# WeeFav/Visual-Odometry-GPU

Measured on AMD Instinct MI355X. Metric: ORB detect+describe frames/sec (1241x376, 8 lvls), higher is better.
Workload: dtype u8; 1 GPU; KITTI-shaped 1241x376 u8, 8 levels s=1.2, 1000 features, FAST-9 t=20, NMS 3x3, Harris top-N, blur5 all levels, BRIEF-256; batch=1024 frames/step/GPU resident in HBM (stream A); distinct_resident_batches=2, fast_early_exit=True, pyramid_blur_fused=True, pyramid_top_rows_first=True, pipelined_batches=True

## Files before the change

visual-odometry-gpu_amd/csrc/orbx_kernels.hip:

```cpp
#include <hip/hip_runtime.h>

#include <cstdlib>

#include "orbx_internal.h"
#include "orbx_math.h"
#include "orbx_wave.h"

__constant__ __attribute__((aligned(16))) int8_t c_pattern[1024] = {
#include "pattern_31.inc"
};


typedef uint16_t __attribute__((aligned(1))) u16_unaligned;

__device__ __forceinline__ void decode_tile(const OrbxTileMap& tm, int nlevels, int& l, int& tx, int& ty) {
  const int t = blockIdx.x;
  l = 0;
#pragma unroll 1
  for (int i = 1; i < nlevels; i++)
    if (t >= tm.begin[i]) l = i;
  const int local = t - tm.begin[l];
  ty = local / tm.tiles_x[l];
  tx = local - ty * tm.tiles_x[l];
}
// ... 705 lines not shown
  const size_t co = (size_t)f * plan.cand_total + L.cand_off;
  const int n8 = (n + 7) & ~7;
  for (int i = tid; i < n8; i += 256) {
    u64 key = 0ull;
    if (i < n) {
      uint32_t u = orbx_f2u(resp[co + i]);
      if (u == 0x80000000u) u = 0u;
      u ^= (u >> 31) ? 0xffffffffu : 0x80000000u;
      key = ((u64)u << 32) | (uint32_t)~(uint32_t)i;
    }
    s_key[i] = key;
  }
  __syncthreads();
  const int ci = tid & (RANK_SLICE - 1), part = tid >> 6;
  const int i = first + ci;
  const u64 ki = s_key[i < n8 ? i : 0];
  const int per = n8 / 4;
  int rank = 0;
  for (int j = part * per; j < (part + 1) * per; j += 2) {
    const ulonglong2 v = *reinterpret_cast<const ulonglong2*>(&s_key[j]);
    rank += v.x > ki;
    rank += v.y > ki;
  }
  s_part[part][ci] = rank;
  __syncthreads();
  if (part == 0 && i < n) {
    rank = s_part[0][ci] + s_part[1][ci] + s_part[2][ci] + s_part[3][ci];
    if (rank < keep) {
      const uint32_t p = cand[co + i];
      const size_t so = (size_t)f * plan.out_cap + L.out_off;
      orbx_keypoint kp;
      kp.x = (int)(p & 0xffffu);
      kp.y = (int)(p >> 16);
      sel_lkp[so + rank] = kp;
      sel_resp[so + rank] = resp[co + i];
    }
  }
}

__global__ __launch_bounds__(256) void k_select_flat(const float* __restrict__ resp, int n, int keep,
                                                     int32_t* __restrict__ idx) {
  const int m = n < keep ? n : keep;
  for (int i = blockIdx.x * 256 + threadIdx.x; i < n; i += gridDim.x * 256) {
    const float ri = resp[i];
    int rank = 0;
    for (int j = 0; j < n; j++) {
      const float rj = resp[j];
      rank += (rj > ri) || (rj == ri && j < i);
    }
    if (rank < m) idx[rank] = i;
  }
}

#define DESC_R 20
#define DESC_ROWS (2 * DESC_R + 1)
#define DESC_PITCH 48
#define DESC_HP 40
#define DESC_BROWS (DESC_ROWS - 4)

struct DescLds {
  union {
    uint32_t patch[DESC_ROWS * DESC_PITCH / 4];
    uint16_t box[DESC_BROWS * DESC_HP];
  };
  uint16_t hs[DESC_ROWS * DESC_HP];
};

__device__ __forceinline__ u64 hsum5x4(uint32_t d0, uint32_t d1) {
  const u64 acc = (u64)__builtin_amdgcn_perm(d1, d1, 0x0c010c00u) |
                  ((u64)__builtin_amdgcn_perm(d1, d1, 0x0c030c02u) << 32);
  return __builtin_amdgcn_qsad_pk_u16_u8((u64)d0 | ((u64)d1 << 32), 0u, acc);
}

struct DescJob {
  const uint8_t* img;
  int w, h, pitch;
  int x, y;
  bool valid;
};

__device__ __forceinline__ void describe_wave(const DescJob& jb, DescLds& lds, int patch_size,
                                              bool use_given_angle, float given_angle, bool do_brief,
                                              float& angle_out, u64 desc_out[4]) {
  const int lane = lane_id();
  const uint8_t* s_patch = reinterpret_cast<const uint8_t*>(lds.patch);
  const int px0 = jb.x - DESC_R, py0 = jb.y - DESC_R;
  const int ax0 = px0 & ~3;
  const int off = px0 - ax0;
  if (jb.valid) {
    int row = lane / (DESC_PITCH / 4), c = lane - row * (DESC_PITCH / 4);
#pragma unroll
    for (int k = 0; k < (DESC_ROWS * (DESC_PITCH / 4) + 63) / 64; k++) {
      const int i = lane + 64 * k;
      if (i < DESC_ROWS * (DESC_PITCH / 4)) {
        const int gy = py0 + row, gx = ax0 + 4 * c;
        uint32_t v = 0;
        if ((unsigned)gy < (unsigned)jb.h && (unsigned)gx < (unsigned)jb.pitch)
          v = *reinterpret_cast<const uint32_t*>(jb.img + (uint32_t)(gy * jb.pitch + gx));
        lds.patch[i] = v;
      }
      row += 5;
      c += 4;
      if (c >= DESC_PITCH / 4) {
        c -= DESC_PITCH / 4;
        row += 1;
      }
    }
  }
  __syncthreads();
  float angle = 0.0f;
  if (jb.valid) {
    if (use_given_angle) {
      angle = given_angle;
    } else {
      const int pr = patch_size / 2, P = 2 * pr + 1;
      if (!(jb.x - pr < 0 || jb.x + pr >= jb.w || jb.y - pr < 0 || jb.y + pr >= jb.h)) {
        const int grp_shift = P <= 32 ? 5 : 6;
        const int col = lane & ((1 << grp_shift) - 1), grp = lane >> grp_shift, ngrp = 64 >> grp_shift;
        int colsum = 0, m01 = 0;
        if (col < P) {
          const uint8_t* pc = s_patch + (DESC_R - pr) * DESC_PITCH + (col - pr + DESC_R + off);
          for (int rr = grp; rr < P; rr += ngrp) {
            const int I = pc[rr * DESC_PITCH];
            colsum += I;
            m01 += (rr - pr) * I;
          }
        }
        int m10 = (col - pr) * colsum;
        m10 = wave_sum(m10);
        m01 = wave_sum(m01);
        angle = orbx_atan2f((float)m01, (float)m10);
      }
    }
  }
  angle_out = angle;
  if (!do_brief) return;

  if (jb.valid) {
    int r = lane / 10, g = lane - r * 10;
#pragma unroll
    for (int k = 0; k < (DESC_ROWS * 10 + 63) / 64; k++) {
      if (lane + 64 * k < DESC_ROWS * 10) {
        const uint32_t d0 = lds.patch[r * (DESC_PITCH / 4) + g], d1 = lds.patch[r * (DESC_PITCH / 4) + g + 1];
        *reinterpret_cast<u64*>(&lds.hs[r * DESC_HP + 4 * g]) = hsum5x4(d0, d1);
      }
      r += 6;
      g += 4;
      if (g >= 10) {
        g -= 10;
        r += 1;
      }
    }
  }
  __syncthreads();
  if (jb.valid) {
    int r = lane / 10, g = lane - r * 10;
#pragma unroll
    for (int k = 0; k < (DESC_BROWS * 10 + 63) / 64; k++) {
      if (lane + 64 * k < DESC_BROWS * 10) {
        const uint2* hp = reinterpret_cast<const uint2*>(&lds.hs[r * DESC_HP + 4 * g]);
        uint2 acc = hp[0];
#pragma unroll
        for (int q = 1; q < 5; q++) {
          const uint2 v = hp[q * (DESC_HP / 4)];
          acc.x = pk_add(acc.x, v.x);
          acc.y = pk_add(acc.y, v.y);
        }
        *reinterpret_cast<uint2*>(&lds.box[r * DESC_HP + 4 * g]) = acc;
      }
      r += 6;
      g += 4;
      if (g >= 10) {
        g -= 10;
        r += 1;
      }
    }
  }
  __syncthreads();

  const float c = orbx_cosf(angle), s = orbx_sinf(angle);
#pragma unroll 1
  for (int k = 0; k < 4; k++) {
    bool bit = false;
    if (jb.valid) {
      const int i = k * 64 + lane;
      const int32_t pk = reinterpret_cast<const int32_t*>(c_pattern)[i];
      const float x1 = (float)(int8_t)(pk & 0xff), y1 = (float)(int8_t)((pk >> 8) & 0xff);
      const float x2 = (float)(int8_t)((pk >> 16) & 0xff), y2 = (float)(int8_t)((pk >> 24) & 0xff);
      int dx1 = orbx_lroundf(__fsub_rn(__fmul_rn(c, x1), __fmul_rn(s, y1)));
      int dy1 = orbx_lroundf(__fadd_rn(__fmul_rn(s, x1), __fmul_rn(c, y1)));
      int dx2 = orbx_lroundf(__fsub_rn(__fmul_rn(c, x2), __fmul_rn(s, y2)));
      int dy2 = orbx_lroundf(__fadd_rn(__fmul_rn(s, x2), __fmul_rn(c, y2)));
      const int cx1 = jb.x + dx1, cy1 = jb.y + dy1, cx2 = jb.x + dx2, cy2 = jb.y + dy2;
      const bool skip = cx1 < 2 || cy1 < 2 || cx1 > jb.w - 1 || cy1 > jb.h - 1 || cx2 < 2 || cy2 < 2 ||
                        cx2 > jb.w - 1 || cy2 > jb.h - 1;
      if (!skip) {
        dx1 = min(max(dx1, -18), 18);
        dy1 = min(max(dy1, -18), 18);
        dx2 = min(max(dx2, -18), 18);
        dy2 = min(max(dy2, -18), 18);
        const int s1 = lds.box[(dy1 + 18) * DESC_HP + dx1 + 18 + off];
        const int s2 = lds.box[(dy2 + 18) * DESC_HP + dx2 + 18 + off];
        bit = s1 < s2;
      }
    }
    desc_out[k] = __ballot(bit);
  }
}



#define DESC_NLD ((DESC_ROWS * (DESC_PITCH / 4) + 63) / 64)

__device__ __forceinline__ void desc_fetch_patch(const DescJob& jb, int lane, uint32_t (&regs)[DESC_NLD],
                                                 int& off_out) {
  const int px0 = jb.x - DESC_R, py0 = jb.y - DESC_R;
  const int ax0 = px0 & ~3;
  off_out = px0 - ax0;
  int row = lane / (DESC_PITCH / 4), c = lane - row * (DESC_PITCH / 4);
#pragma unroll
  for (int k = 0; k < DESC_NLD; k++) {
    const int gy = py0 + row, gx = ax0 + 4 * c;
    uint32_t v = 0;
    if (lane + 64 * k < DESC_ROWS * (DESC_PITCH / 4) && (unsigned)gy < (unsigned)jb.h &&
        (unsigned)gx < (unsigned)jb.pitch)
      v = *reinterpret_cast<const uint32_t*>(jb.img + (uint32_t)(gy * jb.pitch + gx));
    regs[k] = v;
    row += 5;
    c += 4;
    if (c >= DESC_PITCH / 4) {
      c -= DESC_PITCH / 4;
      row += 1;
    }
  }
}

struct DescLds2 {
  uint32_t patch[DESC_ROWS * DESC_PITCH / 4];
  uint16_t hs[DESC_ROWS * DESC_HP];
};

template <class L>
__device__ __forceinline__ void desc_store_patch(L& lds, int lane, const uint32_t (&regs)[DESC_NLD]) {
#pragma unroll
  for (int k = 0; k < DESC_NLD; k++)
    if (lane + 64 * k < DESC_ROWS * (DESC_PITCH / 4)) lds.patch[lane + 64 * k] = regs[k];
}

__device__ __forceinline__ DescJob desc_job(const OrbxPlan& plan, const uint8_t* pyr, int f, orbx_keypoint kp,
                                            int level) {
  const OrbxLevel& L = plan.L[level];
  DescJob jb;
  jb.img = pyr + (size_t)f * plan.frame_bytes + L.img_off;
  jb.w = L.w;
  jb.h = L.h;
  jb.pitch = L.pitch;
  jb.x = kp.x;
  jb.y = kp.y;
  jb.valid = true;
  return jb;
}

template <class L>
__device__ __forceinline__ void desc_box_table_fused(L& lds, int lane) {
  static_assert(DESC_BROWS == 37, "6 chunks: 7 + 5 x 6 rows");
  const int chunk = lane / 10, g = lane - chunk * 10;
  if (chunk < 6) {
    const int r0 = chunk == 0 ? 0 : 6 * chunk + 1, nrows = chunk == 0 ? 7 : 6;
    const uint32_t* pp = &lds.patch[r0 * (DESC_PITCH / 4) + g];
    uint2* bp = reinterpret_cast<uint2*>(&lds.hs[r0 * DESC_HP + 4 * g]);
    auto hrow = [&](int i) {
      const u64 v = hsum5x4(pp[i * (DESC_PITCH / 4)], pp[i * (DESC_PITCH / 4) + 1]);
      return make_uint2((uint32_t)v, (uint32_t)(v >> 32));
    };
    uint2 q[5];
#pragma unroll
    for (int i = 0; i < 5; i++) q[i] = hrow(i);
    uint2 acc;
    acc.x = pk_add(pk_add(pk_add(q[0].x, q[1].x), pk_add(q[2].x, q[3].x)), q[4].x);
    acc.y = pk_add(pk_add(pk_add(q[0].y, q[1].y), pk_add(q[2].y, q[3].y)), q[4].y);
    bp[0] = acc;
#pragma unroll
    for (int i = 1; i < 7; i++) {
      if (i < nrows) {
        const uint2 nw = hrow(i + 4);
        const uint2 od = q[(i - 1) % 5];
        acc.x = pk_sub(pk_add(acc.x, nw.x), od.x);
        acc.y = pk_sub(pk_add(acc.y, nw.y), od.y);
        q[(i - 1) % 5] = nw;
        bp[i * (DESC_HP / 4)] = acc;
      }
    }
  }
  wave_lds_sync();
}

__device__ __forceinline__ float lround_f(float v) {
  const float t = __builtin_truncf(v);
  const float fr = __fsub_rn(v, t);
  return __fadd_rn(t, __builtin_truncf(__fadd_rn(fr, fr)));
}

typedef float f2_t __attribute__((ext_vector_type(2)));
__device__ __forceinline__ f2_t lround_f2(f2_t v) {
  const f2_t t = __builtin_elementwise_trunc(v);
  const f2_t fr = v - t;
  return t + __builtin_elementwise_trunc(fr + fr);
}

template <int DESC_KPW, int DESC_NW, int DESC_OCC>
__global__ __launch_bounds__(64 * DESC_NW, DESC_OCC) void k_describe2(OrbxPlan plan, const uint8_t* __restrict__ pyr, int patch_size,
                                                   const int32_t* __restrict__ sel_count,
                                                   const orbx_keypoint* __restrict__ sel_lkp,
                                                   const float* __restrict__ sel_resp,
                                                   int32_t* __restrict__ out_count,
                                                   orbx_keypoint* __restrict__ out_lkp,
                                                   float* __restrict__ out_resp,
                                                   int32_t* __restrict__ out_level,
                                                   orbx_keypoint* __restrict__ out_kp,
                                                   uint32_t* __restrict__ out_kp16,
                                                   float* __restrict__ out_angle,
                                                   orbx_descriptor* __restrict__ out_desc,
                                                   const uint32_t* __restrict__ feedback, uint32_t* __restrict__ feedback_host,
                                                   OrbxHostRecord host) {
  constexpr int DESC_KPB = DESC_NW * DESC_KPW;
  static_assert(2 * DESC_KPB <= 64 * DESC_NW, "trig: two threads per keypoint");
  __shared__ __attribute__((aligned(16))) DescLds2 s_lds[DESC_NW];
  __shared__ int s_m[DESC_KPB][2];
  __shared__ float s_cs[DESC_KPB][2];
  __shared__ uint2 s_mw[4 * (DESC_PITCH / 4)];
  __shared__ __attribute__((aligned(16))) uint32_t s_rec_kp[DESC_KPB], s_rec_angle[DESC_KPB], s_rec_desc[DESC_KPB][8];
  const int f = blockIdx.x, grp = blockIdx.y, tid = threadIdx.x, lane = tid & 63;
  const int wave = __builtin_amdgcn_readfirstlane(tid >> 6);
  static_assert(ORBX_MAX_LEVELS <= 64, "one lane per level");
  const int lvl_cnt = lane < plan.nlevels ? sel_count[f * plan.nlevels + lane] : 0;
  const int lvl_end = wave_scan_incl(lvl_cnt);
  const int count = __builtin_amdgcn_readlane(lvl_end, 63);
  if (grp == 0 && tid == 0) {
    out_count[f] = count;
    if (host.counts) host.counts[f] = count;
  }
  if (feedback_host && grp == 0 && f == 0 && tid < ORBX_FEEDBACK_WORDS) feedback_host[tid] = feedback[tid];
  const int slot0 = grp * DESC_KPB;
  if (slot0 >= count) return;
  DescLds2& lds = s_lds[wave];
  const int pr = patch_size / 2;
  if (tid < 4 * (DESC_PITCH / 4)) {
    const int off = tid / (DESC_PITCH / 4), c = tid - off * (DESC_PITCH / 4);
    uint32_t xw = 0, on = 0;
#pragma unroll
    for (int b = 0; b < 4; b++) {
      const int t = 4 * c + b - off - (DESC_R - pr);
      if (t >= 0 && t <= 2 * pr) {
        xw |= (uint32_t)t << (8 * b);
        on |= 1u << (8 * b);
      }
    }
    s_mw[tid] = make_uint2(xw, on);
  }
  int rowk[DESC_NLD], c3[3];
  uint32_t rin = 0;
  {
    int row = lane / (DESC_PITCH / 4), c = lane - row * (DESC_PITCH / 4);
#pragma unroll
    for (int k = 0; k < DESC_NLD; k++) {
      rowk[k] = row;
      if (k < 3) c3[k] = c;
      if (lane + 64 * k < DESC_ROWS * (DESC_PITCH / 4) && row >= DESC_R - pr && row <= DESC_R + pr) rin |= 1u << k;
      row += 5;
      c += 4;
      if (c >= DESC_PITCH / 4) {
        c -= DESC_PITCH / 4;
        row += 1;
      }
    }
  }
  __syncthreads();
  const size_t fo = (size_t)f * plan.out_cap;

  const int nk = min(DESC_KPW, max(0, count - (slot0 + wave * DESC_KPW)));
  DescJob jobs[DESC_KPW];
  float scale[DESC_KPW];
  uint32_t regs[DESC_KPW][DESC_NLD];
  int offs[DESC_KPW];
#pragma unroll
  for (int j = 0; j < DESC_KPW; j++) {
    const int slot = min(slot0 + wave * DESC_KPW + j, count - 1);
    const int level = __popcll(__ballot(lvl_end <= slot));
    const int lvl_begin = __builtin_amdgcn_readlane(lvl_end - lvl_cnt, level);
    const size_t src = fo + plan.L[level].out_off + (slot - lvl_begin);
    const orbx_keypoint kp = sel_lkp[src];
    jobs[j] = desc_job(plan, pyr, f, kp, level);
    scale[j] = plan.L[level].scale;
    if (j < nk && lane == 0) {
      out_lkp[fo + slot] = kp;
      out_resp[fo + slot] = sel_resp[src];
      out_level[fo + slot] = level;
    }
  }
#pragma unroll
  for (int j = 0; j < DESC_KPW; j++) {
    const DescJob& jb = jobs[j];
    const int py0 = jb.y - DESC_R, ax0 = (jb.x - DESC_R) & ~3;
    if (py0 >= 0 && py0 + DESC_ROWS <= jb.h && ax0 >= 0 && ax0 + DESC_PITCH <= jb.pitch) {
      offs[j] = jb.x - DESC_R - ax0;
      const uint32_t base = (uint32_t)(py0 * jb.pitch + ax0);
#pragma unroll
      for (int k = 0; k < DESC_NLD; k++) {
        regs[j][k] = 0;
        if (lane + 64 * k < DESC_ROWS * (DESC_PITCH / 4))
          regs[j][k] = *reinterpret_cast<const uint32_t*>(jb.img + (base + (__umul24((uint32_t)rowk[k], (uint32_t)jb.pitch) + 4u * (uint32_t)c3[k % 3])));
      }
    } else {
      desc_fetch_patch(jb, lane, regs[j], offs[j]);
    }
  }

#pragma unroll
  for (int j = 0; j < DESC_KPW; j++) {
    if (j < nk) {
      const DescJob& jb = jobs[j];
      const int q = wave * DESC_KPW + j, off = offs[j];
      int m10 = 0, m01 = 0;
      if (!(jb.x - pr < 0 || jb.x + pr >= jb.w || jb.y - pr < 0 || jb.y + pr >= jb.h)) {
        uint2 mw[3];
#pragma unroll
        for (int m = 0; m < 3; m++) mw[m] = s_mw[off * (DESC_PITCH / 4) + c3[m]];
        uint32_t X = 0, S = 0, M = 0;
#pragma unroll
        for (int k = 0; k < DESC_NLD; k++) {
          const uint32_t z = regs[j][k] & (uint32_t)(-(int32_t)((rin >> k) & 1u));
          X = __builtin_amdgcn_udot4(z, mw[k % 3].x, X, false);
          const uint32_t rs = __builtin_amdgcn_udot4(z, mw[k % 3].y, 0u, false);
          S += rs;
          M += __umul24((uint32_t)rowk[k], rs);
        }
        m10 = wave_sum((int)X - __mul24(pr, (int)S));
        m01 = wave_sum((int)M - __mul24(DESC_R, (int)S));
      }
      if (lane == 0) {
        s_m[q][0] = m10;
        s_m[q][1] = m01;
      }
    }
  }
  __syncthreads();
  if (tid < 2 * DESC_KPB && slot0 + (tid >> 1) < count) {
    const int q = tid >> 1, want_sin = tid & 1;
    const float angle = orbx_atan2f((float)s_m[q][1], (float)s_m[q][0]);
    s_cs[q][want_sin] = orbx_sincosf_impl(angle, want_sin ^ 1);
    if (!want_sin) {
      out_angle[fo + slot0 + q] = angle;
      s_rec_angle[q] = __float_as_uint(angle);
    }
  }
  __syncthreads();

  f2_t patx[4], paty[4];
#pragma unroll
  for (int k = 0; k < 4; k++) {
    const int32_t pk = reinterpret_cast<const int32_t*>(c_pattern)[k * 64 + lane];
    patx[k] = f2_t{(float)(int8_t)(pk & 0xff), (float)(int8_t)((pk >> 16) & 0xff)};
    paty[k] = f2_t{(float)(int8_t)((pk >> 8) & 0xff), (float)(int8_t)((pk >> 24) & 0xff)};
  }
#pragma unroll
  for (int j = 0; j < DESC_KPW; j++) {
    if (j < nk) {
      const DescJob& jb = jobs[j];
      const int q = wave * DESC_KPW + j, slot = slot0 + q, off = offs[j];
      desc_store_patch(lds, lane, regs[j]);
      wave_lds_sync();
      desc_box_table_fused(lds, lane);
      const float c = s_cs[q][0], s = s_cs[q][1];
      const bool interior = jb.x >= DESC_R && jb.y >= DESC_R && jb.x < jb.w - DESC_R && jb.y < jb.h - DESC_R;
      u64 d[4];
      if (interior) {
        const uint16_t* tbl = &lds.hs[18 * DESC_HP + 18 + off];
        const f2_t C2 = {c, c}, S2 = {s, s}, HP2 = {(float)DESC_HP, (float)DESC_HP};
#pragma unroll
        for (int k = 0; k < 4; k++) {
          const f2_t X = patx[k], Y = paty[k];
          const f2_t rx = lround_f2(C2 * X - S2 * Y), ry = lround_f2(S2 * X + C2 * Y);
          const f2_t idx = __builtin_elementwise_fma(ry, HP2, rx);
          d[k] = __ballot(tbl[(int)idx.x] < tbl[(int)idx.y]);
        }
      } else {
#pragma unroll
        for (int k = 0; k < 4; k++) {
          const float x1 = patx[k].x, y1 = paty[k].x, x2 = patx[k].y, y2 = paty[k].y;
          const int dx1 = orbx_lroundf(__fsub_rn(__fmul_rn(c, x1), __fmul_rn(s, y1)));
          const int dy1 = orbx_lroundf(__fadd_rn(__fmul_rn(s, x1), __fmul_rn(c, y1)));
          const int dx2 = orbx_lroundf(__fsub_rn(__fmul_rn(c, x2), __fmul_rn(s, y2)));
          const int dy2 = orbx_lroundf(__fadd_rn(__fmul_rn(s, x2), __fmul_rn(c, y2)));
          const int cx1 = jb.x + dx1, cy1 = jb.y + dy1, cx2 = jb.x + dx2, cy2 = jb.y + dy2;
          const bool ok = !(cx1 < 2 || cy1 < 2 || cx1 > jb.w - 1 || cy1 > jb.h - 1 || cx2 < 2 || cy2 < 2 ||
                            cx2 > jb.w - 1 || cy2 > jb.h - 1);
          const int s1 = lds.hs[(dy1 + 18) * DESC_HP + dx1 + 18 + off];
          const int s2 = lds.hs[(dy2 + 18) * DESC_HP + dx2 + 18 + off];
          d[k] = __ballot(ok && s1 < s2);
        }
      }
      wave_lds_sync();
      if (lane == 0) {
        orbx_keypoint g;
        g.x = (int)__fmul_rn((float)jb.x, scale[j]);
        g.y = (int)__fmul_rn((float)jb.y, scale[j]);
        out_kp[fo + slot] = g;
        out_kp16[fo + slot] = (uint32_t)g.x | ((uint32_t)g.y << 16);
        u64* dd = reinterpret_cast<u64*>(out_desc + fo + slot);
        dd[0] = d[0];
        dd[1] = d[1];
        dd[2] = d[2];
        dd[3] = d[3];
        if (host.desc) {
          s_rec_kp[q] = (uint32_t)g.x | ((uint32_t)g.y << 16);
          u64* sd = reinterpret_cast<u64*>(s_rec_desc[q]);
          sd[0] = d[0];
          sd[1] = d[1];
          sd[2] = d[2];
          sd[3] = d[3];
        }
      }
    }
  }
  if (host.desc) {
    __syncthreads();
    const int nq = min(DESC_KPB, count - slot0);
    if (tid < 2 * nq) {
      const uint4 v = reinterpret_cast<const uint4*>(s_rec_desc[tid >> 1])[tid & 1];
      reinterpret_cast<uint4*>(host.desc + fo + slot0)[tid] = v;
    }
    if (tid < nq) {
      host.kp16[fo + slot0 + tid] = s_rec_kp[tid];
      host.angle[fo + slot0 + tid] = __uint_as_float(s_rec_angle[tid]);
    }
  }
}

__global__ __launch_bounds__(256) void k_describe_flat(const uint8_t* __restrict__ img, int w, int h, int pitch,
                                                       const orbx_keypoint* __restrict__ kps, int nkp,
                                                       int patch_size, int use_given_angles, int do_brief,
                                                       float* __restrict__ angles,
                                                       orbx_descriptor* __restrict__ desc) {
  __shared__ __attribute__((aligned(16))) DescLds s_lds[4];
  const int wave = threadIdx.x >> 6;
  const int slot = blockIdx.x * 4 + wave;
  DescJob jb;
  jb.valid = slot < nkp;
  jb.img = img;
  jb.w = w;
  jb.h = h;
  jb.pitch = pitch;
  jb.x = jb.valid ? kps[slot].x : 0;
  jb.y = jb.valid ? kps[slot].y : 0;
  const float given = (jb.valid && use_given_angles) ? angles[slot] : 0.0f;
  float angle;
  u64 d[4];
  describe_wave(jb, s_lds[wave], patch_size, use_given_angles != 0, given, do_brief != 0, angle, d);
  if (jb.valid && lane_id() == 0) {
    if (!use_given_angles) angles[slot] = angle;
    if (do_brief) {
      u64* dd = reinterpret_cast<u64*>(desc + slot);
      dd[0] = d[0];
      dd[1] = d[1];
      dd[2] = d[2];
      dd[3] = d[3];
    }
  }
}

__global__ __launch_bounds__(256) void k_knn2(const orbx_descriptor* __restrict__ qbase,
                                              const int32_t* __restrict__ qcount, size_t qstride,
                                              const orbx_descriptor* __restrict__ tbase,
                                              const int32_t* __restrict__ tcount, size_t tstride, double ratio,
                                              int32_t* __restrict__ knn_idx, int32_t* __restrict__ knn_dist,
                                              int32_t* __restrict__ match, size_t ostride) {
  __shared__ __attribute__((aligned(16))) uint4 s_t[256 * 2];
  const int p = blockIdx.y, tid = threadIdx.x;
  const int nq = qcount[p], nt = tcount[p];
  if ((int)(blockIdx.x * 256) >= nq) return;
  const int q = blockIdx.x * 256 + tid;
  const bool valid = q < nq;
  const uint4* qp = reinterpret_cast<const uint4*>(qbase + p * qstride + (valid ? q : 0));
  const uint4 qa = qp[0], qb = qp[1];
  const u64 q0 = ((u64)qa.y << 32) | qa.x, q1 = ((u64)qa.w << 32) | qa.z;
  const u64 q2 = ((u64)qb.y << 32) | qb.x, q3 = ((u64)qb.w << 32) | qb.z;
  int d1 = 1 << 30, d2 = 1 << 30, j1 = -1, j2 = -1;
  const orbx_descriptor* tp = tbase + p * tstride;
  for (int t0 = 0; t0 < nt; t0 += 256) {
    const int m = min(256, nt - t0);
    if (tid < m) {
      const uint4* src = reinterpret_cast<const uint4*>(tp + t0 + tid);
      s_t[2 * tid] = src[0];
      s_t[2 * tid + 1] = src[1];
    }
    __syncthreads();
#pragma unroll 4
    for (int j = 0; j < m; j++) {
      const uint4 a = s_t[2 * j], b = s_t[2 * j + 1];
      const int d = __popcll(q0 ^ (((u64)a.y << 32) | a.x)) + __popcll(q1 ^ (((u64)a.w << 32) | a.z)) +
                    __popcll(q2 ^ (((u64)b.y << 32) | b.x)) + __popcll(q3 ^ (((u64)b.w << 32) | b.z));
      if (d < d1) {
        d2 = d1;
        j2 = j1;
        d1 = d;
        j1 = t0 + j;
      } else if (d < d2) {
        d2 = d;
        j2 = t0 + j;
      }
    }
    __syncthreads();
  }
  if (valid) {
    const size_t o = p * ostride + q;
    knn_idx[2 * o] = j1;
    knn_idx[2 * o + 1] = j2;
    knn_dist[2 * o] = j1 >= 0 ? d1 : -1;
    knn_dist[2 * o + 1] = j2 >= 0 ? d2 : -1;
    const bool pass = j2 >= 0 && (double)(float)d1 < ratio * (double)(float)d2;
    match[o] = pass ? j1 : -1;
  }
}


__global__ __launch_bounds__(256) void k_nms_f32(const float* __restrict__ scores, int w, int h, int r,
                                                 float threshold, u64* __restrict__ mask, int mask_wpr) {
  const int y = blockIdx.y * 4 + (threadIdx.x >> 6);
  const int x = blockIdx.x * 64 + (threadIdx.x & 63);
  bool keep = false;
  if (y < h && x < w && !(x < r || y < r || x >= w - r || y >= h - r)) {
    const float v = scores[(size_t)y * w + x];
    keep = v > threshold;
    if (keep)
      for (int dy = -r; dy <= r; dy++)
        for (int dx = -r; dx <= r; dx++) keep = keep && !(scores[(size_t)(y + dy) * w + (x + dx)] > v);
  }
  const u64 m = __ballot(keep);
  if ((threadIdx.x & 63) == 0 && y < h) mask[(size_t)y * mask_wpr + blockIdx.x] = m;
}

__global__ __launch_bounds__(256) void k_conv2d(const uint8_t* __restrict__ img, int w, int h, int pitch,
                                                const float* __restrict__ kern, int K, int reflect_pad,
                                                uint8_t* __restrict__ dst, int dst_pitch) {
  const int wo = reflect_pad ? w : w - K + 1, ho = reflect_pad ? h : h - K + 1;
  const int x = blockIdx.x * 64 + (threadIdx.x & 63), y = blockIdx.y * 4 + (threadIdx.x >> 6);
  if (x >= wo || y >= ho) return;
  const int r = K / 2;
  float sum = 0.f;
  for (int i = 0; i < K; i++)
    for (int j = 0; j < K; j++) {
      int yy, xx;
      if (reflect_pad) {
        yy = reflect101(y - r + i, h);
        xx = reflect101(x - r + j, w);
      } else {
        yy = y + i;
        xx = x + j;
      }
      sum = __fadd_rn(sum, __fmul_rn((float)img[(size_t)yy * pitch + xx], kern[i * K + j]));
    }
  int v = __float2int_rn(sum);
  v = v < 0 ? 0 : (v > 255 ? 255 : v);
  dst[(size_t)y * dst_pitch + x] = (uint8_t)v;
}


#define ORBX_LAUNCH_CHECK() hipGetLastError()

hipError_t orbx_launch_pyramid2(hipStream_t s, const OrbxTileDesc* d_tiles, int n_tiles, int frame_bytes, int w0,
                                int h0, int n_frames, const uint8_t* d_in, int in_stride, size_t in_frame_stride,
                                const OrbxResizeTap* d_taps, uint8_t* d_pyr) {
  if (n_tiles <= 0) return hipSuccess;
  dim3 grid(n_tiles | 1, n_frames);
  hipLaunchKernelGGL(k_pyramid2, grid, dim3(256), 0, s, d_tiles, n_tiles, frame_bytes, w0, h0, d_in, in_stride,
                     in_frame_stride, d_taps, d_pyr);
  return ORBX_LAUNCH_CHECK();
}

hipError_t orbx_launch_blur(hipStream_t s, const OrbxPlan& plan, const OrbxTileMap& tm, int n_frames,
                            const uint8_t* d_src, uint8_t* d_dst, int first_level, int kind) {
  dim3 grid(tm.begin[plan.nlevels], n_frames);
  hipLaunchKernelGGL(k_blur, grid, dim3(256), 0, s, plan, tm, d_src, d_dst, first_level, kind);
  return ORBX_LAUNCH_CHECK();
}

hipError_t orbx_launch_compact(hipStream_t s, const OrbxPlan& plan, int n_frames,
                               const unsigned long long* d_mask, orbx_keypoint* d_cand, int32_t* d_cand_count,
                               int32_t* d_cand_total, int need_total) {
  dim3 grid(plan.nlevels, n_frames);
  hipLaunchKernelGGL(k_compact, grid, dim3(256), 0, s, plan, d_mask, d_cand, d_cand_count, d_cand_total,
                     need_total);
  return ORBX_LAUNCH_CHECK();
}

hipError_t orbx_launch_level_select(hipStream_t s, const OrbxPlan& plan, int n_frames, int mode,
                                    const unsigned long long* d_mask, const uint8_t* d_pyr, const float* d_gauss,
                                    int window, float k, orbx_keypoint* d_sel_lkp, float* d_sel_resp,
                                    int32_t* d_sel_count, uint32_t* d_need) {
  int maxcap = 2;
  for (int l = 0; l < plan.nlevels; l++) maxcap = plan.L[l].cap > maxcap ? plan.L[l].cap : maxcap;
  const size_t lds = (size_t)((maxcap + 1) & ~1) * 16;
  dim3 grid(n_frames, plan.nlevels);
  hipLaunchKernelGGL(k_level_select, grid, dim3(LVL_THREADS), lds, s, plan, mode, d_mask, d_pyr, d_gauss, window, k,
                     d_sel_lkp, d_sel_resp, d_sel_count, d_need);
  return ORBX_LAUNCH_CHECK();
}

hipError_t orbx_launch_level_select_auto(hipStream_t s, const OrbxPlan& plan, int n_frames, int mode, int force,
                                         const unsigned long long* d_mask, const uint8_t* d_pyr,
                                         const float* d_gauss, int window, float k, uint32_t* d_cand,
                                         int32_t* d_ncand, float* d_cresp, orbx_keypoint* d_sel_lkp,
                                         float* d_sel_resp, int32_t* d_sel_count, uint32_t* d_need) {
  int maxcap = 2;
  for (int l = 0; l < plan.nlevels; l++) maxcap = plan.L[l].cap > maxcap ? plan.L[l].cap : maxcap;
  const bool spread = mode == ORBX_SELECT_HARRIS &&
                      (force >= 0 ? force != 0 : maxcap > LVL_THREADS);
  if (!spread)
    return orbx_launch_level_select(s, plan, n_frames, mode, d_mask, d_pyr, d_gauss, window, k, d_sel_lkp,
                                    d_sel_resp, d_sel_count, d_need);
  hipLaunchKernelGGL(k_lvl_compact, dim3(plan.nlevels, n_frames), dim3(256), 0, s, plan, d_mask, d_cand, d_ncand, d_need);
  hipLaunchKernelGGL(k_lvl_harris, dim3((maxcap + 255) / 256, plan.nlevels, n_frames), dim3(256), 0, s, plan, d_pyr,
                     d_gauss, window, k, d_cand, d_ncand, d_cresp);
  const size_t lds = (size_t)((maxcap + 7) & ~7) * 8;
  hipLaunchKernelGGL(k_lvl_rank, dim3((maxcap + RANK_SLICE - 1) / RANK_SLICE, plan.nlevels, n_frames), dim3(256), lds,
                     s, plan, d_cand, d_ncand, d_cresp, d_sel_lkp, d_sel_resp, d_sel_count);
  return ORBX_LAUNCH_CHECK();
}

hipError_t orbx_launch_describe(hipStream_t s, const OrbxPlan& plan, int n_frames, const uint8_t* d_pyr,
                                int patch_size, const int32_t* d_sel_count, const orbx_keypoint* d_sel_lkp,
                                const float* d_sel_resp, int32_t* d_out_count, orbx_keypoint* d_out_lkp,
                                float* d_out_resp, int32_t* d_out_level, orbx_keypoint* d_out_kp, uint32_t* d_out_kp16,
                                float* d_out_angle, orbx_descriptor* d_out_desc, const uint32_t* d_feedback,
                                uint32_t* h_feedback, const OrbxHostRecord* host_record) {
  const OrbxHostRecord host = host_record ? *host_record : OrbxHostRecord{};
  if (plan.out_cap <= 0) return hipSuccess;
  if ((long long)plan.out_cap * n_frames <= 8192) {
    dim3 grid(n_frames, (plan.out_cap + 3) / 4);
    hipLaunchKernelGGL((k_describe2<1, 4, 1>), grid, dim3(256), 0, s, plan, d_pyr, patch_size, d_sel_count, d_sel_lkp,
                       d_sel_resp, d_out_count, d_out_lkp, d_out_resp, d_out_level, d_out_kp, d_out_kp16, d_out_angle, d_out_desc, d_feedback,
                       h_feedback, host);
  } else {
    dim3 grid(n_frames, (plan.out_cap + 15) / 16);
    hipLaunchKernelGGL((k_describe2<4, 4, 6>), grid, dim3(256), 0, s, plan, d_pyr, patch_size, d_sel_count, d_sel_lkp,
                       d_sel_resp, d_out_count, d_out_lkp, d_out_resp, d_out_level, d_out_kp, d_out_kp16, d_out_angle, d_out_desc, d_feedback,
                       h_feedback, host);
  }
  return ORBX_LAUNCH_CHECK();
}

hipError_t orbx_launch_describe_flat(hipStream_t s, const uint8_t* d_img, int w, int h, int pitch,
                                     const orbx_keypoint* d_kps, int nkp, int patch_size, int use_given_angles,
                                     int do_brief, float* d_angles, orbx_descriptor* d_desc) {
  if (nkp <= 0) return hipSuccess;
  hipLaunchKernelGGL(k_describe_flat, dim3((nkp + 3) / 4), dim3(256), 0, s, d_img, w, h, pitch, d_kps, nkp,
                     patch_size, use_given_angles, do_brief, d_angles, d_desc);
  return ORBX_LAUNCH_CHECK();
}

hipError_t orbx_launch_harris_flat(hipStream_t s, const uint8_t* d_img, int w, int h, int pitch,
                                   const orbx_keypoint* d_kps, int nkp, const float* d_gauss, int K, float kk,
                                   float* d_resp) {
  if (nkp <= 0) return hipSuccess;
  hipLaunchKernelGGL(k_harris2_flat, dim3((nkp + 31) / 32), dim3(256), 0, s, d_img, w, h, pitch, d_kps, nkp,
                     d_gauss, K, kk, d_resp);
  return ORBX_LAUNCH_CHECK();
}

hipError_t orbx_launch_nms_f32(hipStream_t s, const float* d_scores, int w, int h, int radius, float threshold,
                               unsigned long long* d_mask, int mask_wpr) {
  dim3 grid((w + 63) / 64, (h + 3) / 4);
  hipLaunchKernelGGL(k_nms_f32, grid, dim3(256), 0, s, d_scores, w, h, radius, threshold, d_mask, mask_wpr);
  return ORBX_LAUNCH_CHECK();
}

hipError_t orbx_launch_conv2d(hipStream_t s, const uint8_t* d_img, int w, int h, int pitch, const float* d_kernel,
                              int K, int reflect_pad, uint8_t* d_dst, int dst_pitch) {
  const int wo = reflect_pad ? w : w - K + 1, ho = reflect_pad ? h : h - K + 1;
  if (wo <= 0 || ho <= 0) return hipSuccess;
  dim3 grid((wo + 63) / 64, (ho + 3) / 4);
  hipLaunchKernelGGL(k_conv2d, grid, dim3(256), 0, s, d_img, w, h, pitch, d_kernel, K, reflect_pad, d_dst,
                     dst_pitch);
  return ORBX_LAUNCH_CHECK();
}

hipError_t orbx_launch_select_flat(hipStream_t s, const float* d_resp, int n, int keep, int32_t* d_idx) {
  if (n <= 0) return hipSuccess;
  int blocks = (n + 255) / 256;
  if (blocks > 1024) blocks = 1024;
  hipLaunchKernelGGL(k_select_flat, dim3(blocks), dim3(256), 0, s, d_resp, n, keep, d_idx);
  return ORBX_LAUNCH_CHECK();
}

hipError_t orbx_launch_knn2(hipStream_t s, int npairs, int max_nq, const orbx_descriptor* d_q, const int32_t* d_qcount,
                            size_t qstride, const orbx_descriptor* d_t, const int32_t* d_tcount, size_t tstride,
                            double ratio, int32_t* d_idx, int32_t* d_dist, int32_t* d_match, size_t ostride) {
  if (npairs <= 0 || max_nq <= 0) return hipSuccess;
  dim3 grid((max_nq + 255) / 256, npairs);
  hipLaunchKernelGGL(k_knn2, grid, dim3(256), 0, s, d_q, d_qcount, qstride, d_t, d_tcount, tstride, ratio, d_idx,
                     d_dist, d_match, ostride);
  return ORBX_LAUNCH_CHECK();
}
```

visual-odometry-gpu_amd/csrc/orbx_math.h:

```cpp
#pragma once
#include <stdint.h>
#include <string.h>

#if defined(__HIPCC__)
#define ORBX_HD __host__ __device__ inline
#else
#define ORBX_HD static inline
#endif

#if defined(__clang__)
#define ORBX_NO_CONTRACT _Pragma("clang fp contract(off)")
#else
#define ORBX_NO_CONTRACT
#endif

ORBX_HD uint32_t orbx_f2u(float f) {
  uint32_t u;
  memcpy(&u, &f, 4);
  return u;
}
ORBX_HD float orbx_u2f(uint32_t u) {
  float f;
  memcpy(&f, &u, 4);
  return f;
}

ORBX_HD float orbx_atanf(float x) {
  ORBX_NO_CONTRACT
  const float atanhi[4] = {(float)4.6364760399e-01, (float)7.8539812565e-01,
                           (float)9.8279368877e-01, (float)1.5707962513e+00};
  const float atanlo[4] = {(float)5.0121582440e-09, (float)3.7748947079e-08,
                           (float)3.4473217170e-08, (float)7.5497894159e-08};
  const float aT0 = (float)3.3333334327e-01, aT1 = (float)-2.0000000298e-01,
              aT2 = (float)1.4285714924e-01, aT3 = (float)-1.1111110449e-01,
              aT4 = (float)9.0908870101e-02, aT5 = (float)-7.6918758452e-02,
              aT6 = (float)6.6610731184e-02, aT7 = (float)-5.8335702866e-02,
              aT8 = (float)4.9768779427e-02, aT9 = (float)-3.6531571299e-02,
              aT10 = (float)1.6285819933e-02;
  const int32_t hx = (int32_t)orbx_f2u(x);
  const int32_t ix = hx & 0x7fffffff;
  int id;
  if (ix >= 0x4c800000) {
    if (ix > 0x7f800000) return x + x;
    float r = atanhi[3] + atanlo[3];
    return hx > 0 ? r : -r;
  }
  if (ix < 0x3ee00000) {
    if (ix < 0x31000000) {
      return x;
    }
    id = -1;
  } else {
    x = orbx_u2f((uint32_t)ix);
    if (ix < 0x3f980000) {
      if (ix < 0x3f300000) {
        id = 0;
        x = (2.0f * x - 1.0f) / (2.0f + x);
      } else {
        id = 1;
        x = (x - 1.0f) / (x + 1.0f);
      }
    } else {
      if (ix < 0x401c0000) {
        id = 2;
        x = (x - 1.5f) / (1.0f + 1.5f * x);
      } else {
        id = 3;
        x = -1.0f / x;
      }
    }
  }
  float z = x * x;
  float w = z * z;
  float s1 = z * (aT0 + w * (aT2 + w * (aT4 + w * (aT6 + w * (aT8 + w * aT10)))));
  float s2 = w * (aT1 + w * (aT3 + w * (aT5 + w * (aT7 + w * aT9))));
  if (id < 0) return x - x * (s1 + s2);
  z = atanhi[id] - ((x * (s1 + s2) - atanlo[id]) - x);
  return hx < 0 ? -z : z;
}

ORBX_HD float orbx_atan2f(float y, float x) {
  ORBX_NO_CONTRACT
  const float tiny = 1.0e-30f;
  const float pi_o_2 = (float)1.5707963705e+00;
  const float pi = (float)3.1415927410e+00;
  const float pi_lo = (float)-8.7422776573e-08;
  const int32_t hx = (int32_t)orbx_f2u(x);
  const int32_t hy = (int32_t)orbx_f2u(y);
  const int32_t ix = hx & 0x7fffffff;
  const int32_t iy = hy & 0x7fffffff;
  if (ix > 0x7f800000 || iy > 0x7f800000) return x + y;
  if (hx == 0x3f800000) return orbx_atanf(y);
  const int m = ((hy >> 31) & 1) | ((hx >> 30) & 2);
  if (iy == 0) {
    switch (m) {
      case 0:
      case 1:
        return y;
      case 2:
        return pi + tiny;
      default:
        return -pi - tiny;
    }
  }
  if (ix == 0) return (hy < 0) ? -pi_o_2 - tiny : pi_o_2 + tiny;
  float z;
  const int32_t k = (iy - ix) >> 23;
  if (k > 60)
    z = pi_o_2 + 0.5f * pi_lo;
  else if (hx < 0 && k < -60)
    z = 0.0f;
  else {
    float q = y / x;
    z = orbx_atanf(orbx_u2f(orbx_f2u(q) & 0x7fffffffu));
  }
  switch (m) {
    case 0:
      return z;
    case 1:
      return orbx_u2f(orbx_f2u(z) ^ 0x80000000u);
    case 2:
      return pi - (z - pi_lo);
    default:
      return (z - pi_lo) - pi;
  }
}

ORBX_HD float orbx_sincos_poly(double x, double x2, int n, int neg_cos) {
  ORBX_NO_CONTRACT
  const double S1 = -0x1.555545995a603p-3, S2 = 0x1.1107605230bc4p-7,
               S3 = -0x1.994eb3774cf24p-13;
  double C0 = 0x1p0, C1 = -0x1.ffffffd0c621cp-2, C2 = 0x1.55553e1068f19p-5,
         C3 = -0x1.6c087e89a359dp-10, C4 = 0x1.99343027bf8c3p-16;
  if (neg_cos) {
    C0 = -C0;
    C1 = -C1;
    C2 = -C2;
    C3 = -C3;
    C4 = -C4;
  }
  if ((n & 1) == 0) {
    double x3 = x * x2;
    double s1 = S2 + x2 * S3;
    double x7 = x3 * x2;
    double s = x + x3 * S1;
    return (float)(s + x7 * s1);
  } else {
    double x4 = x2 * x2;
    double c2 = C3 + x2 * C4;
    double c1 = C0 + x2 * C1;
    double x6 = x4 * x2;
    double c = c1 + x4 * C2;
    return (float)(c + x6 * c2);
  }
}

ORBX_HD uint32_t orbx_abstop12(float x) { return (orbx_f2u(x) >> 20) & 0x7ff; }

ORBX_HD float orbx_sincosf_impl(float y, int want_cos) {
  ORBX_NO_CONTRACT
  const double HPI_INV = 0x1.45F306DC9C883p+23;
  const double HPI = 0x1.921FB54442D18p0;
  const double x = (double)y;
  const uint32_t top = orbx_abstop12(y);
  if (top < orbx_abstop12(0x1.921FB6p-1f)) {
    const double x2 = x * x;
    if (top < orbx_abstop12(0x1p-12f)) return want_cos ? 1.0f : y;
    return orbx_sincos_poly(x, x2, want_cos, 0);
  }
  const double r = x * HPI_INV;
  const int n = ((int32_t)r + 0x800000) >> 24;
  const double xr = x - (double)n * HPI;
  const double sign = ((n & 3) == 1 || (n & 3) == 2) ? -1.0 : 1.0;
  return orbx_sincos_poly(xr * sign, xr * xr, n ^ want_cos, (n & 2) != 0);
}

ORBX_HD float orbx_sinf(float y) { return orbx_sincosf_impl(y, 0); }
ORBX_HD float orbx_cosf(float y) { return orbx_sincosf_impl(y, 1); }

ORBX_HD int orbx_lroundf(float v) {
  ORBX_NO_CONTRACT
  float a = orbx_u2f(orbx_f2u(v) & 0x7fffffffu);
  int t = (int)a;
  float frac = a - (float)t;
  if (frac >= 0.5f) t += 1;
  return ((int32_t)orbx_f2u(v) < 0) ? -t : t;
}
```

visual-odometry-gpu_amd/csrc/orbx_wave.h:

```cpp
#pragma once
#include <hip/hip_runtime.h>
#include <stdint.h>

typedef unsigned long long u64;
typedef unsigned short us2_t __attribute__((ext_vector_type(2)));
typedef short ss2_t __attribute__((ext_vector_type(2)));

__device__ __forceinline__ int lane_id() { return threadIdx.x & 63; }

__device__ __forceinline__ int wave_sum(int v) {
  v += __builtin_amdgcn_update_dpp(0, v, 0xB1 , 0xf, 0xf, true);
  v += __builtin_amdgcn_update_dpp(0, v, 0x4E , 0xf, 0xf, true);
  v += __builtin_amdgcn_update_dpp(0, v, 0x141 , 0xf, 0xf, true);
  v += __builtin_amdgcn_update_dpp(0, v, 0x140 , 0xf, 0xf, true);
  return __builtin_amdgcn_readlane(v, 0) + __builtin_amdgcn_readlane(v, 16) + __builtin_amdgcn_readlane(v, 32) +
         __builtin_amdgcn_readlane(v, 48);
}

__device__ __forceinline__ int wave_scan_incl(int v) {
  const int v0 = v;
  v += __builtin_amdgcn_update_dpp(0, v0, 0x111 , 0xf, 0xf, false);
  v += __builtin_amdgcn_update_dpp(0, v0, 0x112 , 0xf, 0xf, false);
  v += __builtin_amdgcn_update_dpp(0, v0, 0x113 , 0xf, 0xf, false);
  v += __builtin_amdgcn_update_dpp(0, v, 0x114 , 0xf, 0xe, false);
  v += __builtin_amdgcn_update_dpp(0, v, 0x118 , 0xf, 0xc, false);
  v += __builtin_amdgcn_update_dpp(0, v, 0x142 , 0xa, 0xf, false);
  v += __builtin_amdgcn_update_dpp(0, v, 0x143 , 0xc, 0xf, false);
  return v;
}

__device__ __forceinline__ uint32_t pk_add(uint32_t a, uint32_t b) {
  return __builtin_bit_cast(uint32_t, (us2_t)(__builtin_bit_cast(us2_t, a) + __builtin_bit_cast(us2_t, b)));
}
__device__ __forceinline__ uint32_t pk_sub(uint32_t a, uint32_t b) {
  return __builtin_bit_cast(uint32_t, (us2_t)(__builtin_bit_cast(us2_t, a) - __builtin_bit_cast(us2_t, b)));
}
__device__ __forceinline__ uint32_t pk_min_u16(uint32_t a, uint32_t b) {
  return __builtin_bit_cast(uint32_t, __builtin_elementwise_min(__builtin_bit_cast(us2_t, a), __builtin_bit_cast(us2_t, b)));
}
__device__ __forceinline__ uint32_t pk_max_u16(uint32_t a, uint32_t b) {
  return __builtin_bit_cast(uint32_t, __builtin_elementwise_max(__builtin_bit_cast(us2_t, a), __builtin_bit_cast(us2_t, b)));
}
__device__ __forceinline__ uint32_t pk_max_i16(uint32_t a, uint32_t b) {
  return __builtin_bit_cast(uint32_t, __builtin_elementwise_max(__builtin_bit_cast(ss2_t, a), __builtin_bit_cast(ss2_t, b)));
}

__device__ __forceinline__ void wave_lds_sync() {
  __builtin_amdgcn_fence(__ATOMIC_RELEASE, "wavefront");
  __builtin_amdgcn_wave_barrier();
  __builtin_amdgcn_fence(__ATOMIC_ACQUIRE, "wavefront");
}
```

Baseline: 542,200 frames/s.

## Batch moment reductions across keypoints with permlane swaps and coalesce descriptor stores

Replaces the per-keypoint wave_sum reductions for the intensity-centroid moments with a combined transpose-style reduction using permlane32/permlane16 swaps and a 16-lane DPP row sum, so four keypoints share one reduction tree. BRIEF sampling now rounds with a biased add and integer convert instead of trunc-based float rounding, and indexes LDS with an integer multiply. Descriptor and keypoint outputs go through shared memory and are written by many threads at once instead of by lane 0 per keypoint. The risks are rounding differences at exact-half boundaries and a new unconditional block barrier plus staging in the store path.

```diff
diff --git a/visual-odometry-gpu_amd/csrc/orbx_kernels.hip b/visual-odometry-gpu_amd/csrc/orbx_kernels.hip
--- a/visual-odometry-gpu_amd/csrc/orbx_kernels.hip
+++ b/visual-odometry-gpu_amd/csrc/orbx_kernels.hip
@@ -1031,10 +1031,10 @@
 }
 
 typedef float f2_t __attribute__((ext_vector_type(2)));
-__device__ __forceinline__ f2_t lround_f2(f2_t v) {
-  const f2_t t = __builtin_elementwise_trunc(v);
-  const f2_t fr = v - t;
-  return t + __builtin_elementwise_trunc(fr + fr);
+typedef int i2_t __attribute__((ext_vector_type(2)));
+__device__ __forceinline__ i2_t lround_small2(f2_t v) {
+  const f2_t h = {0.5f - 0x1p-25f, 0.5f - 0x1p-25f};
+  return __builtin_convertvector(v + __builtin_elementwise_copysign(h, v), i2_t);
 }
 
 template <int DESC_KPW, int DESC_NW, int DESC_OCC>
@@ -1094,6 +1094,7 @@
 #pragma unroll
     for (int k = 0; k < DESC_NLD; k++) {
       rowk[k] = row;
+      __builtin_assume(row >= 0 && row < DESC_ROWS + 6);
       if (k < 3) c3[k] = c;
       if (lane + 64 * k < DESC_ROWS * (DESC_PITCH / 4) && row >= DESC_R - pr && row <= DESC_R + pr) rin |= 1u << k;
       row += 5;
@@ -1145,31 +1146,50 @@
     }
   }
 
+  int pm[2][DESC_KPW];
 #pragma unroll
   for (int j = 0; j < DESC_KPW; j++) {
-    if (j < nk) {
-      const DescJob& jb = jobs[j];
-      const int q = wave * DESC_KPW + j, off = offs[j];
-      int m10 = 0, m01 = 0;
-      if (!(jb.x - pr < 0 || jb.x + pr >= jb.w || jb.y - pr < 0 || jb.y + pr >= jb.h)) {
-        uint2 mw[3];
-#pragma unroll
-        for (int m = 0; m < 3; m++) mw[m] = s_mw[off * (DESC_PITCH / 4) + c3[m]];
-        uint32_t X = 0, S = 0, M = 0;
-#pragma unroll
-        for (int k = 0; k < DESC_NLD; k++) {
-          const uint32_t z = regs[j][k] & (uint32_t)(-(int32_t)((rin >> k) & 1u));
-          X = __builtin_amdgcn_udot4(z, mw[k % 3].x, X, false);
-          const uint32_t rs = __builtin_amdgcn_udot4(z, mw[k % 3].y, 0u, false);
-          S += rs;
-          M += __umul24((uint32_t)rowk[k], rs);
-        }
-        m10 = wave_sum((int)X - __mul24(pr, (int)S));
-        m01 = wave_sum((int)M - __mul24(DESC_R, (int)S));
-      }
+    const DescJob& jb = jobs[j];
+    const int off = offs[j];
+    pm[0][j] = pm[1][j] = 0;
+    if (j < nk && !(jb.x - pr < 0 || jb.x + pr >= jb.w || jb.y - pr < 0 || jb.y + pr >= jb.h)) {
+      uint2 mw[3];
+#pragma unroll
+      for (int m = 0; m < 3; m++) mw[m] = s_mw[off * (DESC_PITCH / 4) + c3[m]];
+      uint32_t X = 0, S = 0, M = 0;
+#pragma unroll
+      for (int k = 0; k < DESC_NLD; k++) {
+        const uint32_t z = regs[j][k] & (uint32_t)(-(int32_t)((rin >> k) & 1u));
+        X = __builtin_amdgcn_udot4(z, mw[k % 3].x, X, false);
+        const uint32_t rs = __builtin_amdgcn_udot4(z, mw[k % 3].y, 0u, false);
+        S += rs;
+        M += __umul24((uint32_t)rowk[k], rs);
+      }
+      pm[0][j] = (int)X - __mul24(pr, (int)S);
+      pm[1][j] = (int)M - __mul24(DESC_R, (int)S);
+    }
+  }
+  if constexpr (DESC_KPW == 4) {
+    int u[2];
+#pragma unroll
+    for (int i = 0; i < 2; i++) {
+      const auto h0 = __builtin_amdgcn_permlane32_swap(pm[i][0], pm[i][1], false, false);
+      const auto h1 = __builtin_amdgcn_permlane32_swap(pm[i][2], pm[i][3], false, false);
+      const auto r = __builtin_amdgcn_permlane16_swap(h0[0] + h0[1], h1[0] + h1[1], false, false);
+      u[i] = row_sum16(r[0] + r[1]);
+    }
+    if ((lane & 15) == 0) {
+      const int q = wave * DESC_KPW + (((lane >> 4) & 1) << 1 | (lane >> 5));
+      s_m[q][0] = u[0];
+      s_m[q][1] = u[1];
+    }
+  } else {
+#pragma unroll
+    for (int j = 0; j < DESC_KPW; j++) {
+      const int m10 = wave_sum(pm[0][j]), m01 = wave_sum(pm[1][j]);
       if (lane == 0) {
-        s_m[q][0] = m10;
-        s_m[q][1] = m01;
+        s_m[wave * DESC_KPW + j][0] = m10;
+        s_m[wave * DESC_KPW + j][1] = m01;
       }
     }
   }
@@ -1196,7 +1216,7 @@
   for (int j = 0; j < DESC_KPW; j++) {
     if (j < nk) {
       const DescJob& jb = jobs[j];
-      const int q = wave * DESC_KPW + j, slot = slot0 + q, off = offs[j];
+      const int q = wave * DESC_KPW + j, off = offs[j];
       desc_store_patch(lds, lane, regs[j]);
       wave_lds_sync();
       desc_box_table_fused(lds, lane);
@@ -1205,13 +1225,17 @@
       u64 d[4];
       if (interior) {
         const uint16_t* tbl = &lds.hs[18 * DESC_HP + 18 + off];
-        const f2_t C2 = {c, c}, S2 = {s, s}, HP2 = {(float)DESC_HP, (float)DESC_HP};
+        auto at = [&](int x, int y) {
+          int i = __mul24(y, DESC_HP) + x;
+          asm("" : "+v"(i));
+          return tbl[i];
+        };
+        const f2_t C2 = {c, c}, S2 = {s, s};
 #pragma unroll
         for (int k = 0; k < 4; k++) {
           const f2_t X = patx[k], Y = paty[k];
-          const f2_t rx = lround_f2(C2 * X - S2 * Y), ry = lround_f2(S2 * X + C2 * Y);
-          const f2_t idx = __builtin_elementwise_fma(ry, HP2, rx);
-          d[k] = __ballot(tbl[(int)idx.x] < tbl[(int)idx.y]);
+          const i2_t rx = lround_small2(C2 * X - S2 * Y), ry = lround_small2(S2 * X + C2 * Y);
+          d[k] = __ballot(at(rx.x, ry.x) < at(rx.y, ry.y));
         }
       } else {
 #pragma unroll
@@ -1231,36 +1255,32 @@
       }
       wave_lds_sync();
       if (lane == 0) {
-        orbx_keypoint g;
-        g.x = (int)__fmul_rn((float)jb.x, scale[j]);
-        g.y = (int)__fmul_rn((float)jb.y, scale[j]);
-        out_kp[fo + slot] = g;
-        out_kp16[fo + slot] = (uint32_t)g.x | ((uint32_t)g.y << 16);
-        u64* dd = reinterpret_cast<u64*>(out_desc + fo + slot);
-        dd[0] = d[0];
-        dd[1] = d[1];
-        dd[2] = d[2];
-        dd[3] = d[3];
-        if (host.desc) {
-          s_rec_kp[q] = (uint32_t)g.x | ((uint32_t)g.y << 16);
-          u64* sd = reinterpret_cast<u64*>(s_rec_desc[q]);
-          sd[0] = d[0];
-          sd[1] = d[1];
-          sd[2] = d[2];
-          sd[3] = d[3];
-        }
-      }
-    }
-  }
-  if (host.desc) {
-    __syncthreads();
-    const int nq = min(DESC_KPB, count - slot0);
-    if (tid < 2 * nq) {
-      const uint4 v = reinterpret_cast<const uint4*>(s_rec_desc[tid >> 1])[tid & 1];
-      reinterpret_cast<uint4*>(host.desc + fo + slot0)[tid] = v;
-    }
-    if (tid < nq) {
-      host.kp16[fo + slot0 + tid] = s_rec_kp[tid];
+        const int gx = (int)__fmul_rn((float)jb.x, scale[j]), gy = (int)__fmul_rn((float)jb.y, scale[j]);
+        s_rec_kp[q] = (uint32_t)gx | ((uint32_t)gy << 16);
+        u64* sd = reinterpret_cast<u64*>(s_rec_desc[q]);
+        sd[0] = d[0];
+        sd[1] = d[1];
+        sd[2] = d[2];
+        sd[3] = d[3];
+      }
+    }
+  }
+  __syncthreads();
+  const int nq = min(DESC_KPB, count - slot0);
+  if (tid < 2 * nq) {
+    const uint4 v = reinterpret_cast<const uint4*>(s_rec_desc[tid >> 1])[tid & 1];
+    reinterpret_cast<uint4*>(out_desc + fo + slot0)[tid] = v;
+    if (host.desc) reinterpret_cast<uint4*>(host.desc + fo + slot0)[tid] = v;
+  }
+  if (tid < nq) {
+    const uint32_t kp16 = s_rec_kp[tid];
+    orbx_keypoint g;
+    g.x = (int)(kp16 & 0xffffu);
+    g.y = (int)(kp16 >> 16);
+    out_kp[fo + slot0 + tid] = g;
+    out_kp16[fo + slot0 + tid] = kp16;
+    if (host.desc) {
+      host.kp16[fo + slot0 + tid] = kp16;
       host.angle[fo + slot0 + tid] = __uint_as_float(s_rec_angle[tid]);
     }
   }
diff --git a/visual-odometry-gpu_amd/csrc/orbx_math.h b/visual-odometry-gpu_amd/csrc/orbx_math.h
--- a/visual-odometry-gpu_amd/csrc/orbx_math.h
+++ b/visual-odometry-gpu_amd/csrc/orbx_math.h
@@ -186,3 +186,9 @@
   if (frac >= 0.5f) t += 1;
   return ((int32_t)orbx_f2u(v) < 0) ? -t : t;
 }
+
+ORBX_HD float orbx_lround_biased(float v) {
+  ORBX_NO_CONTRACT
+  return v + __builtin_copysignf(0.5f - 0x1p-25f, v);
+}
+ORBX_HD int orbx_lround_small(float v) { return (int)orbx_lround_biased(v); }
diff --git a/visual-odometry-gpu_amd/csrc/orbx_wave.h b/visual-odometry-gpu_amd/csrc/orbx_wave.h
--- a/visual-odometry-gpu_amd/csrc/orbx_wave.h
+++ b/visual-odometry-gpu_amd/csrc/orbx_wave.h
@@ -8,11 +8,16 @@
 
 __device__ __forceinline__ int lane_id() { return threadIdx.x & 63; }
 
-__device__ __forceinline__ int wave_sum(int v) {
+__device__ __forceinline__ int row_sum16(int v) {
   v += __builtin_amdgcn_update_dpp(0, v, 0xB1 , 0xf, 0xf, true);
   v += __builtin_amdgcn_update_dpp(0, v, 0x4E , 0xf, 0xf, true);
   v += __builtin_amdgcn_update_dpp(0, v, 0x141 , 0xf, 0xf, true);
   v += __builtin_amdgcn_update_dpp(0, v, 0x140 , 0xf, 0xf, true);
+  return v;
+}
+
+__device__ __forceinline__ int wave_sum(int v) {
+  v = row_sum16(v);
   return __builtin_amdgcn_readlane(v, 0) + __builtin_amdgcn_readlane(v, 16) + __builtin_amdgcn_readlane(v, 32) +
          __builtin_amdgcn_readlane(v, 48);
 }
```

Measured after the change: 552,600 frames/s, median of 6. 1.02x the previous value.
